# Kyubyong/dc_tts

Hardware: NVIDIA H100
Metric: mel_frames_per_sec (higher is better)
Workload: dtype f32 (decode: fp32 FMA; TextEnc/SSRN: fp16x2 split operands on wgmma, fp32 accumulate)

## Files before the change

### dc_tts_b200/csrc/api_synth.cu

```cuda
#include "api_internal.cuh"

namespace {

size_t decode_plane_halfs(H* h, int B, __half* base = nullptr, DecParams* set = nullptr) {
    const int T = h->hp.max_T;
    const std::vector<int> rows = audiodec_rows(h->audiodec, T);
    size_t off = 0;
    for (size_t i = 1; i < rows.size() && rows[i] > 1; ++i) {
        if (set) set->pl_hist[set->n_enc + i] = base + off;
        off += (size_t)B * h->audiodec[i].cin * 2 * (DEC_PL_PAD + T);
    }
    if (set) { set->pl_c1 = base + off; set->pl_rows = DEC_PL_PAD + T; }
    if (!h->audiodec.empty()) off += (size_t)(B + DEC_GMAX) * h->audiodec[0].cin * 2 * DEC_PL_PAD;
    return off;
}

}

void dctts::api::settle_decode_counts(H* h) {
    auto& D = h->dec;
    if (D.last_clusters > 0 && (D.last_moved_frames < 0 || D.frames_pending)) CUDA_CHECK(cudaDeviceSynchronize());
    if (D.last_clusters > 0 && D.last_moved_frames < 0) {
        std::vector<int> st(2 * (size_t)D.last_clusters);
        CUDA_CHECK(cudaMemcpy(st.data(), D.stats.p, st.size() * sizeof(int), cudaMemcpyDeviceToHost));
// ... 219 lines not shown
    }
    a.stages = std::min((occ2 || win.jptr) ? 2 : tc_stages_for(p.bn, bk, a.resid_tma, a.half), std::max(1, a.ntaps * a.kb_per_tap));
    if (debug)
        fprintf(stderr, "[tc] %s mode=%d ncta=%d bn=%d half=%d stages=%d nkb=%d tiles=%d TT=%d TB=%d L=%d B=%d\n", l.scope.c_str(),
                a.mode, p.ncta, a.bn, a.half, a.stages, a.ntaps * a.kb_per_tap, tiles, TT, TB, win.L, win.B);
    launch_conv_ln_tc(mAh, mAl, mWh, mWl, a.resid_tma ? io : nullptr, a, p.ncta, tiles, bk, lc.s); lc.count();
    if (debug) {
        cudaError_t e = cudaStreamSynchronize(lc.s);
        for (int c = 0; c < std::min(16, p.ncta * tiles); ++c)
            fprintf(stderr, "[tc]  cta %2d: start=%d tmem=0x%x nkb=%d tma=%d mma=%d acc_ready=%d published=%d combined=%d\n", c,
                    dbg_host[64 * c], dbg_host[64 * c + 1], dbg_host[64 * c + 2], dbg_host[64 * c + 3], dbg_host[64 * c + 4],
                    dbg_host[64 * c + 5], dbg_host[64 * c + 6], dbg_host[64 * c + 7]);
        {
            const int* d0 = dbg_host;
            auto dt = [&](int a_, int b_) { return (d0[b_] - d0[a_]) & 0x7fffffff; };
            fprintf(stderr, "[tc]  cta 0 cycles: setup %d | main loop %d | sweeps1+2 %d | cluster barrier %d | sweep3+stores %d | teardown %d | total %d\n",
                    dt(8, 9), dt(9, 10), dt(10, 11), dt(11, 12), dt(12, 13), dt(13, 14), dt(8, 14));
        }
        if (e != cudaSuccess) throw std::runtime_error(std::string("conv_ln_tc failed: ") + cudaGetErrorString(e));
    }
}

bool chain_tc_ok(H* h, const std::vector<LayerDev>& net) {
    if (h->tensor_path != 1) return false;
    for (auto& l : net) if (!l.tc.ok) return false;
    return true;
}

void run_chain_tc_planes(Launch& lc, const std::vector<LayerDev>& net, Planes cur, int which, int B, int L,
                         float* out, float* out_sig, int first_extra_shift, const float* in_inv, const int* lengths) {
    H* h = lc.h;
// ... 624 lines not shown
```

### dc_tts_b200/csrc/kernels_tc.cu

```cuda
#include "kernels_tc.cuh"
#include "numerics.cuh"
#include "tc_ptx.cuh"

#include <cstdlib>
#include <stdexcept>
#include <string>

namespace dctts {

using namespace ptx;

constexpr int TC_BM = 128;
constexpr int TC_THREADS = 384;
constexpr int TC_MAX_STAGES = 8;
constexpr int TC_AUX_BYTES = 256  + 3 * 512 * 4  + 128 * 16 ;
constexpr int TC_MAX_SMEM = 227 * 1024;

__device__ __forceinline__ void dbg_mark(int* dbg, int slot, int v) {
    if (dbg) {
        const int cta = blockIdx.y * gridDim.x + blockIdx.x;
        if (cta < 16) { reinterpret_cast<volatile int*>(dbg)[64 * cta + slot] = v; __threadfence_system(); }
    }
}

__device__ __forceinline__ void dbg_time(int* dbg, int slot) {
    if (dbg) dbg_mark(dbg, slot, (int)(clock64() & 0x7fffffff));
}

__device__ __forceinline__ void store_planes(const Planes& p, size_t row, int col, int C, const float (&o)[16]) {
    __half* hi = p.hi + row * p.ld + col;
    __half* lo = p.lo + row * p.ld + col;
    if (col + 16 <= p.ld) {
        split_store_f16<16>(o, hi, lo);
    } else {
#pragma unroll
        for (int i = 0; i < 16; ++i)
            if (col + i < C) split_f16(o[i], hi[i], lo[i]);
    }
}

__host__ __device__ inline int tc_acc_ld(int bn) { return bn + 4; }
__host__ __device__ inline int tc_ring_bytes(int stages, int stage_bytes, int bn) {
    const int ring = stages * stage_bytes;
    const int acc = TC_BM * tc_acc_ld(bn) * 4;
    return ((ring > acc ? ring : acc) + 1023) & ~1023;
}
__host__ __device__ constexpr int tc_max_cluster(int bn) { return bn == 144 ? 16 : 8; }
__host__ __device__ inline int tc_resid_bytes(int resid_tma, int half) { return resid_tma ? 2 * (half / 64) * 16384 : 0; }

template <int TC_BK, int BN>
__global__ void __launch_bounds__(TC_THREADS, 1)
conv_ln_tc_kernel(const __grid_constant__ CUtensorMap mapA_hi, const __grid_constant__ CUtensorMap mapA_lo,
                  const __grid_constant__ CUtensorMap mapW_hi, const __grid_constant__ CUtensorMap mapW_lo,
                  const __grid_constant__ CUtensorMap mapX_hi, const __grid_constant__ CUtensorMap mapX_lo,
                  const __grid_constant__ CUtensorMap mapO_hi, const __grid_constant__ CUtensorMap mapO_lo,
                  const TcArgs a) {
    extern __shared__ uint8_t smem_raw[];
    uint8_t* smem = reinterpret_cast<uint8_t*>((reinterpret_cast<uintptr_t>(smem_raw) + 1023) & ~uintptr_t(1023));
    pdl_launch_dependents();

    const int warp = threadIdx.x >> 5, lane = threadIdx.x & 31;
    const int wg = threadIdx.x >> 7;
    const bool epi = wg == 1;
    if (threadIdx.x == 0) dbg_time(a.dbg, 8);
    const int rank = (int)cluster_ctarank();
    const int ncta = (int)cluster_nctarank();
    const int nslices = ncta;
    constexpr int MAXC = tc_max_cluster(BN);
    constexpr int bn = BN;
    const int half = a.half;
    constexpr int TC_A_PLANE = TC_BM * TC_BK * 2;
    constexpr int SW = TC_BK * 2;
    constexpr int b_plane = bn * SW;
    constexpr int A_BYTES = 2 * TC_A_PLANE;
    constexpr int stage_bytes = A_BYTES + 2 * b_plane;
    const int stages = a.stages;
    const int nkb = a.ntaps * a.kb_per_tap;
    const int acc_ld = tc_acc_ld(bn);

    float* s_acc = reinterpret_cast<float*>(smem);
    uint8_t* rs = smem + tc_ring_bytes(stages, stage_bytes, bn);
    uint8_t* aux = rs + tc_resid_bytes(a.resid_tma, half);
    uint64_t* full_bar = reinterpret_cast<uint64_t*>(aux);
    uint64_t* empty_bar = full_bar + TC_MAX_STAGES;
    uint64_t* resid_bar = empty_bar + TC_MAX_STAGES;
    float* s_bias = reinterpret_cast<float*>(aux + 256);
    float* s_gam = s_bias + 512;
    float* s_bet = s_gam + 512;
    float4* s_part = reinterpret_cast<float4*>(s_bet + 512);

    pdl_wait();
    const int L = a.win.L;
    int t_end, t_lo;
    if (a.win.jptr) { t_end = __ldg(a.win.jptr); t_lo = max(0, t_end - a.win.R + 1); }
    else { t_end = L - 1; t_lo = 0; }
    int b0s, t0s;
// ... 19 lines not shown
        } else {
            int second = c >= half;
            int col = rank * half + (second ? c - half : c);
            bi = (a.mode == 1 && second) ? a.bias[a.C + col] : a.bias[col];
            g = second ? a.g2[col] : a.g1[col];
            be = second ? a.b2[col] : a.b1[col];
        }
        s_bias[c] = bi; s_gam[c] = g; s_bet[c] = be;
    }
    __syncthreads();
    if (threadIdx.x == 0) { dbg_mark(a.dbg, 0, 1); dbg_mark(a.dbg, 2, nkb); dbg_time(a.dbg, 9); }
    if (ncta > 1) { cluster_arrive(); cluster_wait(); }
    const uint16_t cta_mask = (uint16_t)((1u << ncta) - 1u);
    const int slice_rows = TC_BM / ncta;

    if (warp == 0) {
        if (lane == 0) {
            for (int kb = 0; kb < nkb; ++kb) {
                const int s = kb % stages;
                const uint32_t ph = (uint32_t)(kb / stages) & 1u;
                mbar_wait(&empty_bar[s], ph ^ 1u);
                mbar_expect_tx(&full_bar[s], (uint32_t)stage_bytes);
                uint8_t* st = smem + (size_t)s * stage_bytes;
                const int tap = kb / a.kb_per_tap, kc = kb - tap * a.kb_per_tap;
                const int tcoord = t0s + a.shifts[tap];
                if (mcast) {
                    const int off = rank * slice_rows * SW;
                    tma_load_3d_mc(&mapA_hi, &full_bar[s], st + off, kc * TC_BK, tcoord + rank * slice_rows, b0s, cta_mask);
                    tma_load_3d_mc(&mapA_lo, &full_bar[s], st + TC_A_PLANE + off, kc * TC_BK, tcoord + rank * slice_rows, b0s, cta_mask);
                } else {
                    tma_load_3d(&mapA_hi, &full_bar[s], st, kc * TC_BK, tcoord, b0s);
                    tma_load_3d(&mapA_lo, &full_bar[s], st + TC_A_PLANE, kc * TC_BK, tcoord, b0s);
                }
                tma_load_2d(&mapW_hi, &full_bar[s], st + A_BYTES, kb * TC_BK, rank * bn);
                tma_load_2d(&mapW_lo, &full_bar[s], st + A_BYTES + b_plane, kb * TC_BK, rank * bn);
            }
            dbg_mark(a.dbg, 3, nkb);
            if (a.resid_tma) {
                const int nbox = half / 64;
                mbar_expect_tx(resid_bar, (uint32_t)(2 * nbox * 16384));
                for (int i = 0; i < nbox; ++i) {
                    tma_load_3d(&mapX_hi, resid_bar, rs + i * 16384, rank * half + i * 64, t0s, b0s);
                    tma_load_3d(&mapX_lo, resid_bar, rs + (nbox + i) * 16384, rank * half + i * 64, t0s, b0s);
                }
            }
        }
        __syncwarp();
    } else if (wg >= 1) {
        const int mh = wg - 1;
        float acc[BN / 2];
#pragma unroll
        for (int i = 0; i < BN / 2; ++i) acc[i] = 0.f;
        auto release = [&](int s) {
            const int t = threadIdx.x & 127;
            if (mcast) { if (t < ncta) mbar_arrive_cluster(&empty_bar[s], (uint32_t)t); }
            else if (t == 0) mbar_arrive(&empty_bar[s]);
        };
        for (int kb = 0; kb < nkb; ++kb) {
            const int s = kb % stages;
            mbar_wait(&full_bar[s], (uint32_t)(kb / stages) & 1u);
            const uint32_t st = smem_u32(smem + (size_t)s * stage_bytes);
            const uint64_t dA_hi = gmma_desc_kmajor<SW>(st + mh * 64 * SW), dA_lo = gmma_desc_kmajor<SW>(st + TC_A_PLANE + mh * 64 * SW);
            const uint64_t dB_hi = gmma_desc_kmajor<SW>(st + A_BYTES), dB_lo = gmma_desc_kmajor<SW>(st + A_BYTES + b_plane);
            wg_fence();
#pragma unroll
            for (int k = 0; k < TC_BK / 16; ++k) {
                const uint64_t adv = (uint64_t)(k * 32 >> 4);
                wgmma_full<BN>(acc, dA_hi + adv, dB_hi + adv, (kb | k) != 0);
                wgmma_full<BN>(acc, dA_hi + adv, dB_lo + adv, 1u);
                wgmma_full<BN>(acc, dA_lo + adv, dB_hi + adv, 1u);
            }
            wg_commit();
            wg_wait<1>();
            if (kb > 0) release((kb - 1) % stages);
        }
        wg_wait<0>();
        wg_fence_regs(acc);
        if (threadIdx.x == 128) dbg_mark(a.dbg, 4, nkb);
        named_sync(1, 256);
        {
            const int w4 = (threadIdx.x >> 5) & 3;
            const int r0 = mh * 64 + w4 * 16 + (lane >> 2);
#pragma unroll
            for (int q = 0; q < BN / 8; ++q) {
                const int col = q * 8 + 2 * (lane & 3);
                *reinterpret_cast<float2*>(s_acc + (size_t)r0 * acc_ld + col) = make_float2(acc[q * 4], acc[q * 4 + 1]);
                *reinterpret_cast<float2*>(s_acc + (size_t)(r0 + 8) * acc_ld + col) = make_float2(acc[q * 4 + 2], acc[q * 4 + 3]);
            }
        }
        named_sync(1, 256);
    }
    if (epi) {
        const int r = threadIdx.x - 128;
        const float* arow = s_acc + (size_t)r * acc_ld;
        auto ld16 = [&](int c, float (&v)[16]) {
#pragma unroll
            for (int i = 0; i < 16; i += 4) {
                const float4 x = *reinterpret_cast<const float4*>(arow + c + i);
                v[i] = x.x; v[i + 1] = x.y; v[i + 2] = x.z; v[i + 3] = x.w;
            }
        };
        const int bi = r / a.TT, ti = r - bi * a.TT;
        const int n1 = (a.mode == 0) ? min(max(a.C - rank * bn, 0), bn) : half;
        if (r == 0) { dbg_mark(a.dbg, 5, 1); dbg_time(a.dbg, 10); }

        const int b = b0s + bi, t = t0s + ti;
        const bool row_ok = (b < a.win.B) && (t >= t_lo) && (t <= t_end) && (t < L);
        const bool live = !(a.lengths && b < a.win.B) ||
                          t < (min(max(__ldg(a.lengths + b), 0), L >> a.len_shift) << a.len_shift);
        const float in_s = (a.in_inv && b < a.win.B) ? __ldg(a.in_inv + b) : 1.f;
        const float inv_s = a.inv_scale * in_s;

        float s1, s2 = 0.f, q1, q2 = 0.f, m1, m2 = 0.f;
        {
            float piv = 0.f, S = 0.f, Q = 0.f;
            for (int c = 0; c < n1; c += 16) {
                float v[16];
                ld16(c, v);
                if (c == 0) piv = fmaf(v[0], inv_s, s_bias[0]);
#pragma unroll
                for (int i = 0; i < 16; ++i) {
                    const int cc = c + i;
                    if (cc < n1) { const float d = fmaf(v[i], inv_s, s_bias[cc]) - piv; S += d; Q = fmaf(d, d, Q); }
                }
            }
            const float n = (float)max(n1, 1);
            s1 = piv * (float)n1 + S; m1 = n1 > 0 ? s1 / n : 0.f; q1 = fmaxf(Q - S * S / n, 0.f);
        }
        if (a.mode != 0) {
            float piv = 0.f, S = 0.f, Q = 0.f;
            for (int c = 0; c < half; c += 16) {
                float v[16];
                ld16(half + c, v);
                if (c == 0) piv = fmaf(v[0], inv_s, s_bias[half]);
#pragma unroll
                for (int i = 0; i < 16; ++i) {
                    const int cc = c + i;
                    if (cc < half) { const float d = fmaf(v[i], inv_s, s_bias[half + cc]) - piv; S += d; Q = fmaf(d, d, Q); }
                }
            }
            s2 = piv * (float)half + S; m2 = s2 / (float)half; q2 = fmaxf(Q - S * S / (float)half, 0.f);
        }
        float mean1, rstd1, mean2 = 0.f, rstd2 = 0.f;
        if (ncta > 1) {
            s_part[r] = make_float4(s1, q1, s2, q2);
            if (r == 0) { dbg_mark(a.dbg, 6, 1); dbg_time(a.dbg, 11); }
            cluster_arrive();
            cluster_wait();
            if (r == 0) { dbg_mark(a.dbg, 7, 1); dbg_time(a.dbg, 12); }
            const uint32_t my_slot = smem_u32(&s_part[r]);
            float4 pv[MAXC];
#pragma unroll
            for (int p = 0; p < MAXC; ++p) pv[p] = (p < nslices) ? ld_cluster_f4(mapa(my_slot, (uint32_t)p)) : make_float4(0.f, 0.f, 0.f, 0.f);
            float S1 = 0.f, S2 = 0.f;
#pragma unroll
            for (int p = 0; p < MAXC; ++p) if (p < nslices) { S1 += pv[p].x; S2 += pv[p].z; }
            mean1 = S1 / (float)a.C; mean2 = S2 / (float)a.C;
            float M1 = 0.f, M2 = 0.f;
#pragma unroll
            for (int p = 0; p < MAXC; ++p) {
                if (p >= nslices) continue;
                const float4 v = pv[p];
                const int np = (a.mode == 0) ? min(max(a.C - p * bn, 0), bn) : half;
                if (np > 0) { float d = v.x / (float)np - mean1; M1 += v.y + (float)np * d * d; }
                if (a.mode != 0) { float d = v.z / (float)half - mean2; M2 += v.w + (float)half * d * d; }
            }
            rstd1 = 1.0f / sqrtf(M1 / (float)a.C + 1e-12f);
            rstd2 = 1.0f / sqrtf(M2 / (float)a.C + 1e-12f);
        } else {
            mean1 = m1; rstd1 = 1.0f / sqrtf(q1 / (float)a.C + 1e-12f);
            mean2 = m2; rstd2 = 1.0f / sqrtf(q2 / (float)a.C + 1e-12f);
        }

        {
            if (a.mode == 0) {
                const size_t row = (size_t)b * L + t;
                for (int c = 0; c < n1; c += 16) {
                    float v[16], o[16];
                    ld16(c, v);
                    const int col = rank * bn + c;
#pragma unroll
                    for (int i = 0; i < 16; ++i) {
                        float z = (fmaf(v[i], inv_s, s_bias[c + i]) - mean1) * rstd1 * s_gam[c + i] + s_bet[c + i];
                        if (a.act == 1) z = fmaxf(z, 0.f);
                        o[i] = (c + i < n1 && live) ? z : 0.f;
                    }
                    if (row_ok && a.out.hi) store_planes(a.out, row, col, a.C, o);
                    if (row_ok && a.out_f32) {
                        float* p = a.out_f32 + row * a.ld_f32 + col;
#pragma unroll
                        for (int i = 0; i < 16; ++i) if (c + i < n1) p[i] = o[i];
                    }
                    if (a.sig_f32 || a.sig.hi) {
#pragma unroll
                        for (int i = 0; i < 16; ++i) o[i] = (c + i < n1 && live) ? sigmoid_acc(o[i]) : 0.f;
                        if (row_ok && a.sig.hi) store_planes(a.sig, row, col, a.C, o);
                        if (row_ok && a.sig_f32) {
                            float* p = a.sig_f32 + row * a.ld_sig + col;
#pragma unroll
                            for (int i = 0; i < 16; ++i) if (c + i < n1) p[i] = o[i];
                        }
                    }
                }
            } else if (a.mode == 1) {
                const size_t row = (size_t)b * L + t;
                const int nbox = half / 64;
                if (a.resid_tma) mbar_wait(resid_bar, 0);
                for (int c = 0; c < half; c += 16) {
                    float v1[16], v2[16], o[16];
                    const int col = rank * half + c;
                    __align__(16) __half xh[16] = {};
                    __align__(16) __half xl[16] = {};
                    uint8_t* sh = rs + (c >> 6) * 16384 + r * 128;
                    uint8_t* sl = sh + nbox * 16384;
                    const int k0 = (((c & 63) >> 3) ^ (r & 7)) << 4, k1 = ((((c & 63) >> 3) + 1) ^ (r & 7)) << 4;
                    if (a.resid_tma) {
                        reinterpret_cast<uint4*>(xh)[0] = *reinterpret_cast<const uint4*>(sh + k0);
                        reinterpret_cast<uint4*>(xh)[1] = *reinterpret_cast<const uint4*>(sh + k1);
                        reinterpret_cast<uint4*>(xl)[0] = *reinterpret_cast<const uint4*>(sl + k0);
                        reinterpret_cast<uint4*>(xl)[1] = *reinterpret_cast<const uint4*>(sl + k1);
                    } else if (row_ok) {
                        const uint4* ph = reinterpret_cast<const uint4*>(a.X.hi + row * a.X.ld + col);
                        const uint4* pl = reinterpret_cast<const uint4*>(a.X.lo + row * a.X.ld + col);
                        reinterpret_cast<uint4*>(xh)[0] = __ldg(ph); reinterpret_cast<uint4*>(xh)[1] = __ldg(ph + 1);
                        reinterpret_cast<uint4*>(xl)[0] = __ldg(pl); reinterpret_cast<uint4*>(xl)[1] = __ldg(pl + 1);
                    }
                    ld16(c, v1);
                    ld16(half + c, v2);
#pragma unroll
                    for (int i = 0; i < 16; ++i) {
                        float z1 = (fmaf(v1[i], inv_s, s_bias[c + i]) - mean1) * rstd1 * s_gam[c + i] + s_bet[c + i];
                        float z2 = (fmaf(v2[i], inv_s, s_bias[half + c + i]) - mean2) * rstd2 * s_gam[half + c + i] + s_bet[half + c + i];
                        float h1 = sigmoid_acc(z1);
                        float x = join_f16(xh[i], xl[i]);
                        o[i] = live ? h1 * z2 + (1.0f - h1) * x : 0.f;
                    }
                    if (a.out_tma) {
                        __align__(16) __half oh[16];
                        __align__(16) __half ol[16];
#pragma unroll
                        for (int i = 0; i < 16; ++i) split_f16(o[i], oh[i], ol[i]);
                        *reinterpret_cast<uint4*>(sh + k0) = reinterpret_cast<const uint4*>(oh)[0];
                        *reinterpret_cast<uint4*>(sh + k1) = reinterpret_cast<const uint4*>(oh)[1];
                        *reinterpret_cast<uint4*>(sl + k0) = reinterpret_cast<const uint4*>(ol)[0];
                        *reinterpret_cast<uint4*>(sl + k1) = reinterpret_cast<const uint4*>(ol)[1];
                    } else if (row_ok && a.out.hi) {
                        store_planes(a.out, row, col, a.C, o);
                    }
                    if (row_ok && a.out_f32) {
                        float* p = a.out_f32 + row * a.ld_f32 + col;
#pragma unroll
                        for (int i = 0; i < 16; ++i) p[i] = o[i];
                    }
                }
                if (a.out_tma) {
                    fence_proxy_async_smem();
                    named_sync(2, 128);
                    if (r == 0) {
                        for (int i = 0; i < nbox; ++i) {
                            tma_store_3d(&mapO_hi, rs + i * 16384, rank * half + i * 64, t0s, b0s);
                            tma_store_3d(&mapO_lo, rs + (nbox + i) * 16384, rank * half + i * 64, t0s, b0s);
                        }
                        tma_store_commit_and_wait();
                    }
                }
            } else {
                const size_t row_e = (size_t)b * (2 * L) + 2 * (size_t)t;
                for (int hsel = 0; hsel < 2; ++hsel) {
                    const float mean = hsel ? mean2 : mean1, rstd = hsel ? rstd2 : rstd1;
                    for (int c = 0; c < half; c += 16) {
                        float v[16], o[16];
                        ld16(hsel * half + c, v);
                        const int col = rank * half + c;
#pragma unroll
                        for (int i = 0; i < 16; ++i) {
                            const int ac = hsel * half + c + i;
                            o[i] = live ? (fmaf(v[i], inv_s, s_bias[ac]) - mean) * rstd * s_gam[ac] + s_bet[ac] : 0.f;
                        }
                        if (row_ok && a.out.hi) store_planes(a.out, row_e + hsel, col, a.C, o);
                        if (row_ok && a.out_f32) {
                            float* p = a.out_f32 + (row_e + hsel) * a.ld_f32 + col;
#pragma unroll
                            for (int i = 0; i < 16; ++i) p[i] = o[i];
                        }
                    }
                }
            }
        }
        if (r == 0) dbg_time(a.dbg, 13);
    }

    if (ncta > 1) {
        if (!epi) { cluster_arrive(); cluster_wait(); }
        cluster_arrive();
        cluster_wait();
    }
    if (threadIdx.x == 0) dbg_time(a.dbg, 14);
}

__global__ void f32_to_planes_kernel(const float* __restrict__ x, int ldx, Planes p, long long rows, int C) {
    long long i = (long long)blockIdx.x * blockDim.x + threadIdx.x;
    long long total = rows * C;
    if (i >= total) return;
    long long r = i / C; int c = (int)(i - r * C);
    split_f16(x[r * ldx + c], p.hi[r * p.ld + c], p.lo[r * p.ld + c]);
}
__global__ void planes_to_f32_kernel(Planes p, float* __restrict__ y, int ldy, long long rows, int C) {
    long long i = (long long)blockIdx.x * blockDim.x + threadIdx.x;
// ... 94 lines not shown
    cuuint64_t strides[1] = {(cuuint64_t)Ktot * 2};
    cuuint32_t box[2] = {(cuuint32_t)bk, (cuuint32_t)bn};
    cuuint32_t estr[2] = {1, 1};
    CUresult r = encode_fn()(m, CU_TENSOR_MAP_DATA_TYPE_FLOAT16, 2, const_cast<__half*>(base), dims, strides, box, estr,
                             CU_TENSOR_MAP_INTERLEAVE_NONE, bk == 64 ? CU_TENSOR_MAP_SWIZZLE_128B : CU_TENSOR_MAP_SWIZZLE_64B, CU_TENSOR_MAP_L2_PROMOTION_L2_256B,
                             CU_TENSOR_MAP_FLOAT_OOB_FILL_NONE);
    if (r != CUDA_SUCCESS) throw std::runtime_error("cuTensorMapEncodeTiled(weights) failed: " + std::to_string((int)r));
}

int tc_bk() {
    return 32;
}

static size_t conv_ln_smem(int stages, int bn, int half, int resid_tma, int bk) {
    const int stage = 2 * TC_BM * bk * 2 + 2 * bn * bk * 2;
    return (size_t)tc_ring_bytes(stages, stage, bn) + tc_resid_bytes(resid_tma, half) + TC_AUX_BYTES + 1024;
}

int tc_stages_for(int bn, int bk, int resid_tma, int half) {
    int s = TC_MAX_STAGES;
    while (s > 2 && conv_ln_smem(s, bn, half, resid_tma, bk) > (size_t)TC_MAX_SMEM) --s;
    return s;
}

typedef void (*ConvLnKernel)(const CUtensorMap, const CUtensorMap, const CUtensorMap, const CUtensorMap, const CUtensorMap,
                             const CUtensorMap, const CUtensorMap, const CUtensorMap, const TcArgs);
template <int BK>
static ConvLnKernel conv_ln_kernel_bn(int bn) {
    switch (bn) {
        case 64: return conv_ln_tc_kernel<BK, 64>;
        case 80: return conv_ln_tc_kernel<BK, 80>;
// ... 29 lines not shown
    cudaLaunchAttribute at[1];
    at[0].id = cudaLaunchAttributeClusterDimension;
    at[0].val.clusterDim.x = (unsigned)ncta; at[0].val.clusterDim.y = 1; at[0].val.clusterDim.z = 1;
    cfg.attrs = at; cfg.numAttrs = 1;
    int n = 0;
    if (cudaOccupancyMaxActiveClusters(&n, kern, &cfg) != cudaSuccess) { cudaGetLastError(); return 0; }
    return n;
}

void launch_conv_ln_tc(const CUtensorMap& a_hi, const CUtensorMap& a_lo, const CUtensorMap& w_hi,
                       const CUtensorMap& w_lo, const CUtensorMap* io, const TcArgs& a, int ncta, int ctas_y, int bk,
                       cudaStream_t s) {
    if (ncta > tc_max_cluster(a.bn))
        throw std::runtime_error("conv_ln_tc: a cluster of " + std::to_string(ncta) + " CTAs at " + std::to_string(a.bn) +
                                 " columns (16 at 144 columns, else 8 at most)");
    const ConvLnKernel kern = conv_ln_kernel_ready(bk, a.bn);
    const size_t smem = conv_ln_smem(a.stages, a.bn, a.half, a.resid_tma, bk);
    if (smem > (size_t)TC_MAX_SMEM) throw std::runtime_error("conv_ln_tc: shared memory budget exceeded");
    cudaLaunchConfig_t cfg{};
    cfg.gridDim = dim3((unsigned)ncta, (unsigned)ctas_y, 1);
    cfg.blockDim = dim3(TC_THREADS, 1, 1);
    cfg.dynamicSmemBytes = smem;
    cfg.stream = s;
    cudaLaunchAttribute at[2];
    at[0].id = cudaLaunchAttributeClusterDimension;
    at[0].val.clusterDim.x = (unsigned)ncta; at[0].val.clusterDim.y = 1; at[0].val.clusterDim.z = 1;
    at[1].id = cudaLaunchAttributeProgrammaticStreamSerialization;
    at[1].val.programmaticStreamSerializationAllowed = 1;
    cfg.attrs = at; cfg.numAttrs = pdl_enabled() ? 2 : 1;
    if (a.resid_tma && !io) throw std::runtime_error("conv_ln_tc: residual TMA needs the X / out tensor maps");
// ... 10 lines not shown
```

### dc_tts_b200/csrc/tc_ptx.cuh

```cuda
#pragma once
#include <cuda_runtime.h>
#include <stdint.h>

namespace dctts { namespace ptx {

__device__ __forceinline__ uint32_t smem_u32(const void* p) {
    return static_cast<uint32_t>(__cvta_generic_to_shared(p));
}
__device__ __forceinline__ bool elect_one() {
    uint32_t pred = 0;
    asm volatile("{\n\t.reg .pred P;\n\telect.sync _|P, 0xffffffff;\n\tselp.u32 %0, 1, 0, P;\n\t}" : "=r"(pred));
    return pred != 0;
}

__device__ __forceinline__ void mbar_init(uint64_t* bar, uint32_t count) {
    asm volatile("mbarrier.init.shared::cta.b64 [%0], %1;" :: "r"(smem_u32(bar)), "r"(count));
}
__device__ __forceinline__ void fence_mbar_init() { asm volatile("fence.mbarrier_init.release.cluster;" ::: "memory"); }
__device__ __forceinline__ void mbar_expect_tx(uint64_t* bar, uint32_t bytes) {
    asm volatile("mbarrier.arrive.expect_tx.shared::cta.b64 _, [%0], %1;" :: "r"(smem_u32(bar)), "r"(bytes) : "memory");
}
__device__ __forceinline__ bool mbar_try_wait(uint64_t* bar, uint32_t parity) {
    uint32_t ok;
    asm volatile(
// ... 130 lines not shown
    return d;
}

__device__ __forceinline__ void mbar_arrive(uint64_t* bar) {
    asm volatile("mbarrier.arrive.shared::cta.b64 _, [%0];" :: "r"(smem_u32(bar)) : "memory");
}
__device__ __forceinline__ uint32_t mapa(uint32_t smem_addr, uint32_t rank);
__device__ __forceinline__ void mbar_arrive_cluster(uint64_t* bar, uint32_t rank) {
    asm volatile("mbarrier.arrive.release.cluster.shared::cluster.b64 _, [%0];" :: "r"(mapa(smem_u32(bar), rank)) : "memory");
}
__device__ __forceinline__ void mbar_arrive_remote(uint64_t* bar, uint32_t rank) {
    asm volatile("mbarrier.arrive.shared::cluster.b64 _, [%0];" :: "r"(mapa(smem_u32(bar), rank)) : "memory");
}
__device__ __forceinline__ void named_sync(int id, int n) { asm volatile("bar.sync %0, %1;" :: "r"(id), "r"(n) : "memory"); }

__device__ __forceinline__ uint32_t cluster_ctarank() { uint32_t r; asm volatile("mov.u32 %0, %%cluster_ctarank;" : "=r"(r)); return r; }
__device__ __forceinline__ uint32_t cluster_nctarank() { uint32_t r; asm volatile("mov.u32 %0, %%cluster_nctarank;" : "=r"(r)); return r; }
__device__ __forceinline__ void cluster_arrive() { asm volatile("barrier.cluster.arrive.release.aligned;" ::: "memory"); }
__device__ __forceinline__ void cluster_wait() { asm volatile("barrier.cluster.wait.acquire.aligned;" ::: "memory"); }
__device__ __forceinline__ uint32_t mapa(uint32_t smem_addr, uint32_t rank) {
    uint32_t r;
    asm volatile("mapa.shared::cluster.u32 %0, %1, %2;" : "=r"(r) : "r"(smem_addr), "r"(rank));
    return r;
}
__device__ __forceinline__ float4 ld_cluster_f4(uint32_t addr) {
    float4 v;
    asm volatile("ld.shared::cluster.v4.f32 {%0, %1, %2, %3}, [%4];" : "=f"(v.x), "=f"(v.y), "=f"(v.z), "=f"(v.w) : "r"(addr) : "memory");
    return v;
}
__device__ __forceinline__ void st_cluster_f4(uint32_t addr, float a, float b, float c, float d) {
// ... 5 lines not shown
```

Measured before the change: 136,800.

## Compute LayerNorm epilogue directly from wgmma register fragments instead of smem staging

The conv+LayerNorm tensor-core kernel used to dump its accumulators to a shared-memory tile and have one warpgroup redo row statistics and normalisation per row. Now both MMA warpgroups apply bias, compute row statistics with quad shuffles, normalise and store directly from their register fragments. Stores use quad transposes to form 16-byte writes. This removes the smem round trip and the accumulator tile from the smem budget, which may allow more pipeline stages. Register reallocation via setmaxnreg gives the consumer warpgroups more registers; it adds shuffle work and a new constraint that hc/transposed modes need half == bn/2.

```diff
diff --git a/dc_tts_b200/csrc/api_synth.cu b/dc_tts_b200/csrc/api_synth.cu
--- a/dc_tts_b200/csrc/api_synth.cu
+++ b/dc_tts_b200/csrc/api_synth.cu
@@ -257,7 +257,7 @@
         {
             const int* d0 = dbg_host;
             auto dt = [&](int a_, int b_) { return (d0[b_] - d0[a_]) & 0x7fffffff; };
-            fprintf(stderr, "[tc]  cta 0 cycles: setup %d | main loop %d | sweeps1+2 %d | cluster barrier %d | sweep3+stores %d | teardown %d | total %d\n",
+            fprintf(stderr, "[tc]  cta 0 cycles: setup %d | main loop %d | statistics %d | cluster barrier %d | normalise+stores %d | teardown %d | total %d\n",
                     dt(8, 9), dt(9, 10), dt(10, 11), dt(11, 12), dt(12, 13), dt(13, 14), dt(8, 14));
         }
         if (e != cudaSuccess) throw std::runtime_error(std::string("conv_ln_tc failed: ") + cudaGetErrorString(e));
diff --git a/dc_tts_b200/csrc/kernels_tc.cu b/dc_tts_b200/csrc/kernels_tc.cu
--- a/dc_tts_b200/csrc/kernels_tc.cu
+++ b/dc_tts_b200/csrc/kernels_tc.cu
@@ -27,24 +27,82 @@
     if (dbg) dbg_mark(dbg, slot, (int)(clock64() & 0x7fffffff));
 }
 
-__device__ __forceinline__ void store_planes(const Planes& p, size_t row, int col, int C, const float (&o)[16]) {
-    __half* hi = p.hi + row * p.ld + col;
-    __half* lo = p.lo + row * p.ld + col;
-    if (col + 16 <= p.ld) {
-        split_store_f16<16>(o, hi, lo);
-    } else {
-#pragma unroll
-        for (int i = 0; i < 16; ++i)
-            if (col + i < C) split_f16(o[i], hi[i], lo[i]);
-    }
-}
-
-__host__ __device__ inline int tc_acc_ld(int bn) { return bn + 4; }
-__host__ __device__ inline int tc_ring_bytes(int stages, int stage_bytes, int bn) {
-    const int ring = stages * stage_bytes;
-    const int acc = TC_BM * tc_acc_ld(bn) * 4;
-    return ((ring > acc ? ring : acc) + 1023) & ~1023;
-}
+
+template <int G0, int NG, int R>
+__device__ __forceinline__ void row_stats(const float (&v)[R], int h, int j, int n, float& s, float& m2) {
+    const float piv = __shfl_sync(0xffffffffu, v[4 * G0 + 2 * h], (threadIdx.x & 31) & ~3);
+    float S = 0.f, Q = 0.f;
+#pragma unroll
+    for (int k = 0; k < NG; ++k)
+#pragma unroll
+        for (int e = 0; e < 2; ++e)
+            if (8 * k + 2 * j + e < n) { const float d = v[4 * (G0 + k) + 2 * h + e] - piv; S += d; Q = fmaf(d, d, Q); }
+#pragma unroll
+    for (int m = 1; m < 4; m <<= 1) { S += __shfl_xor_sync(0xffffffffu, S, m); Q += __shfl_xor_sync(0xffffffffu, Q, m); }
+    s = piv * (float)n + S;
+    m2 = fmaxf(Q - S * S / (float)max(n, 1), 0.f);
+}
+
+__device__ __forceinline__ void quad_transpose(uint32_t (&x)[4], int j) {
+#pragma unroll
+    for (int m = 2; m > 0; m >>= 1) {
+        const bool up = (j & m) != 0;
+#pragma unroll
+        for (int k = 0; k < 4; ++k) {
+            if (k & m) continue;
+            const uint32_t r = __shfl_xor_sync(0xffffffffu, up ? x[k] : x[k ^ m], m);
+            if (up) x[k] = r; else x[k ^ m] = r;
+        }
+    }
+}
+
+__device__ __forceinline__ uint32_t h2_bits(__half2 v) { return *reinterpret_cast<uint32_t*>(&v); }
+
+template <int G0, int NG, int R>
+__device__ __forceinline__ void store_planes_frag(const Planes& p, size_t row, int col0, const float (&v)[R], int h, int j,
+                                                  bool ok) {
+    __half* hi = p.hi + row * p.ld;
+    __half* lo = p.lo + row * p.ld;
+#pragma unroll
+    for (int k = 0; k + 4 <= NG; k += 4) {
+        uint32_t xh[4], xl[4];
+#pragma unroll
+        for (int i = 0; i < 4; ++i) {
+            const int q = G0 + k + i;
+            __half2 a, b;
+            split_f16x2(make_float2(v[4 * q + 2 * h], v[4 * q + 2 * h + 1]), a, b);
+            xh[i] = h2_bits(a); xl[i] = h2_bits(b);
+        }
+        quad_transpose(xh, j);
+        quad_transpose(xl, j);
+        const int col = col0 + 8 * (k + j);
+        if (ok && col + 8 <= p.ld) {
+            *reinterpret_cast<uint4*>(hi + col) = make_uint4(xh[0], xh[1], xh[2], xh[3]);
+            *reinterpret_cast<uint4*>(lo + col) = make_uint4(xl[0], xl[1], xl[2], xl[3]);
+        }
+    }
+#pragma unroll
+    for (int k = NG & ~3; k < NG; ++k) {
+        const int q = G0 + k, col = col0 + 8 * k + 2 * j;
+        __half2 a, b;
+        split_f16x2(make_float2(v[4 * q + 2 * h], v[4 * q + 2 * h + 1]), a, b);
+        if (ok && col + 2 <= p.ld) { *reinterpret_cast<__half2*>(hi + col) = a; *reinterpret_cast<__half2*>(lo + col) = b; }
+    }
+}
+
+template <int G0, int NG, int R>
+__device__ __forceinline__ void store_f32_frag(float* dst, int col0, int n, const float (&v)[R], int h, int j) {
+#pragma unroll
+    for (int k = 0; k < NG; ++k) {
+        const int c = 8 * k + 2 * j;
+        const float x0 = v[4 * (G0 + k) + 2 * h], x1 = v[4 * (G0 + k) + 2 * h + 1];
+        float* d = dst + col0 + c;
+        if (c + 1 < n && (reinterpret_cast<uintptr_t>(d) & 7) == 0) *reinterpret_cast<float2*>(d) = make_float2(x0, x1);
+        else { if (c < n) d[0] = x0; if (c + 1 < n) d[1] = x1; }
+    }
+}
+
+__host__ __device__ inline int tc_ring_bytes(int stages, int stage_bytes) { return (stages * stage_bytes + 1023) & ~1023; }
 __host__ __device__ constexpr int tc_max_cluster(int bn) { return bn == 144 ? 16 : 8; }
 __host__ __device__ inline int tc_resid_bytes(int resid_tma, int half) { return resid_tma ? 2 * (half / 64) * 16384 : 0; }
 
@@ -56,12 +114,11 @@
                   const __grid_constant__ CUtensorMap mapO_hi, const __grid_constant__ CUtensorMap mapO_lo,
                   const TcArgs a) {
     extern __shared__ uint8_t smem_raw[];
-    uint8_t* smem = reinterpret_cast<uint8_t*>((reinterpret_cast<uintptr_t>(smem_raw) + 1023) & ~uintptr_t(1023));
+    uint8_t* smem = smem_raw + ((1024u - (smem_u32(smem_raw) & 1023u)) & 1023u);
     pdl_launch_dependents();
 
     const int warp = threadIdx.x >> 5, lane = threadIdx.x & 31;
     const int wg = threadIdx.x >> 7;
-    const bool epi = wg == 1;
     if (threadIdx.x == 0) dbg_time(a.dbg, 8);
     const int rank = (int)cluster_ctarank();
     const int ncta = (int)cluster_nctarank();
@@ -69,6 +126,7 @@
     constexpr int MAXC = tc_max_cluster(BN);
     constexpr int bn = BN;
     const int half = a.half;
+    constexpr int HALF = BN / 2, NG = BN / 8, HG = BN / 16;
     constexpr int TC_A_PLANE = TC_BM * TC_BK * 2;
     constexpr int SW = TC_BK * 2;
     constexpr int b_plane = bn * SW;
@@ -76,10 +134,8 @@
     constexpr int stage_bytes = A_BYTES + 2 * b_plane;
     const int stages = a.stages;
     const int nkb = a.ntaps * a.kb_per_tap;
-    const int acc_ld = tc_acc_ld(bn);
-
-    float* s_acc = reinterpret_cast<float*>(smem);
-    uint8_t* rs = smem + tc_ring_bytes(stages, stage_bytes, bn);
+
+    uint8_t* rs = smem + tc_ring_bytes(stages, stage_bytes);
     uint8_t* aux = rs + tc_resid_bytes(a.resid_tma, half);
     uint64_t* full_bar = reinterpret_cast<uint64_t*>(aux);
     uint64_t* empty_bar = full_bar + TC_MAX_STAGES;
@@ -129,8 +185,9 @@
     const uint16_t cta_mask = (uint16_t)((1u << ncta) - 1u);
     const int slice_rows = TC_BM / ncta;
 
-    if (warp == 0) {
-        if (lane == 0) {
+    if (wg == 0) {
+        setmaxnreg_dec<40>();
+        if (warp == 0 && lane == 0) {
             for (int kb = 0; kb < nkb; ++kb) {
                 const int s = kb % stages;
                 const uint32_t ph = (uint32_t)(kb / stages) & 1u;
@@ -161,7 +218,8 @@
             }
         }
         __syncwarp();
-    } else if (wg >= 1) {
+    } else {
+        setmaxnreg_inc<232>();
         const int mh = wg - 1;
         float acc[BN / 2];
 #pragma unroll
@@ -191,222 +249,197 @@
         }
         wg_wait<0>();
         wg_fence_regs(acc);
-        if (threadIdx.x == 128) dbg_mark(a.dbg, 4, nkb);
-        named_sync(1, 256);
-        {
-            const int w4 = (threadIdx.x >> 5) & 3;
-            const int r0 = mh * 64 + w4 * 16 + (lane >> 2);
-#pragma unroll
-            for (int q = 0; q < BN / 8; ++q) {
-                const int col = q * 8 + 2 * (lane & 3);
-                *reinterpret_cast<float2*>(s_acc + (size_t)r0 * acc_ld + col) = make_float2(acc[q * 4], acc[q * 4 + 1]);
-                *reinterpret_cast<float2*>(s_acc + (size_t)(r0 + 8) * acc_ld + col) = make_float2(acc[q * 4 + 2], acc[q * 4 + 3]);
-            }
-        }
-        named_sync(1, 256);
-    }
-    if (epi) {
-        const int r = threadIdx.x - 128;
-        const float* arow = s_acc + (size_t)r * acc_ld;
-        auto ld16 = [&](int c, float (&v)[16]) {
-#pragma unroll
-            for (int i = 0; i < 16; i += 4) {
-                const float4 x = *reinterpret_cast<const float4*>(arow + c + i);
-                v[i] = x.x; v[i + 1] = x.y; v[i + 2] = x.z; v[i + 3] = x.w;
-            }
-        };
-        const int bi = r / a.TT, ti = r - bi * a.TT;
-        const int n1 = (a.mode == 0) ? min(max(a.C - rank * bn, 0), bn) : half;
-        if (r == 0) { dbg_mark(a.dbg, 5, 1); dbg_time(a.dbg, 10); }
-
-        const int b = b0s + bi, t = t0s + ti;
-        const bool row_ok = (b < a.win.B) && (t >= t_lo) && (t <= t_end) && (t < L);
-        const bool live = !(a.lengths && b < a.win.B) ||
-                          t < (min(max(__ldg(a.lengths + b), 0), L >> a.len_shift) << a.len_shift);
-        const float in_s = (a.in_inv && b < a.win.B) ? __ldg(a.in_inv + b) : 1.f;
-        const float inv_s = a.inv_scale * in_s;
-
-        float s1, s2 = 0.f, q1, q2 = 0.f, m1, m2 = 0.f;
-        {
-            float piv = 0.f, S = 0.f, Q = 0.f;
-            for (int c = 0; c < n1; c += 16) {
-                float v[16];
-                ld16(c, v);
-                if (c == 0) piv = fmaf(v[0], inv_s, s_bias[0]);
-#pragma unroll
-                for (int i = 0; i < 16; ++i) {
-                    const int cc = c + i;
-                    if (cc < n1) { const float d = fmaf(v[i], inv_s, s_bias[cc]) - piv; S += d; Q = fmaf(d, d, Q); }
-                }
-            }
-            const float n = (float)max(n1, 1);
-            s1 = piv * (float)n1 + S; m1 = n1 > 0 ? s1 / n : 0.f; q1 = fmaxf(Q - S * S / n, 0.f);
-        }
-        if (a.mode != 0) {
-            float piv = 0.f, S = 0.f, Q = 0.f;
-            for (int c = 0; c < half; c += 16) {
-                float v[16];
-                ld16(half + c, v);
-                if (c == 0) piv = fmaf(v[0], inv_s, s_bias[half]);
-#pragma unroll
-                for (int i = 0; i < 16; ++i) {
-                    const int cc = c + i;
-                    if (cc < half) { const float d = fmaf(v[i], inv_s, s_bias[half + cc]) - piv; S += d; Q = fmaf(d, d, Q); }
-                }
-            }
-            s2 = piv * (float)half + S; m2 = s2 / (float)half; q2 = fmaxf(Q - S * S / (float)half, 0.f);
-        }
-        float mean1, rstd1, mean2 = 0.f, rstd2 = 0.f;
+        if (threadIdx.x == 128) { dbg_mark(a.dbg, 4, nkb); dbg_mark(a.dbg, 5, 1); dbg_time(a.dbg, 10); }
+
+        const int j = lane & 3;
+        const int rt = mh * 64 + (warp & 3) * 16 + (lane >> 2);
+        int bb[2], tt[2];
+        bool ok[2], live[2];
+        float inv_s[2];
+#pragma unroll
+        for (int h = 0; h < 2; ++h) {
+            const int r = rt + 8 * h, bi = r / a.TT;
+            const int b = b0s + bi, t = t0s + r - bi * a.TT;
+            bb[h] = b; tt[h] = t;
+            ok[h] = (b < a.win.B) && (t >= t_lo) && (t <= t_end) && (t < L);
+            live[h] = !(a.lengths && b < a.win.B) || t < (min(max(__ldg(a.lengths + b), 0), L >> a.len_shift) << a.len_shift);
+            inv_s[h] = a.inv_scale * ((a.in_inv && b < a.win.B) ? __ldg(a.in_inv + b) : 1.f);
+        }
+#pragma unroll
+        for (int q = 0; q < NG; ++q) {
+            const float2 bi2 = *reinterpret_cast<const float2*>(s_bias + 8 * q + 2 * j);
+#pragma unroll
+            for (int h = 0; h < 2; ++h) {
+                acc[4 * q + 2 * h] = fmaf(acc[4 * q + 2 * h], inv_s[h], bi2.x);
+                acc[4 * q + 2 * h + 1] = fmaf(acc[4 * q + 2 * h + 1], inv_s[h], bi2.y);
+            }
+        }
+        const int n1 = (a.mode == 0) ? min(max(a.C - rank * bn, 0), bn) : HALF;
+
+        float s1[2], q1[2], s2[2] = {0.f, 0.f}, q2[2] = {0.f, 0.f};
+#pragma unroll
+        for (int h = 0; h < 2; ++h) {
+            if (a.mode == 0) row_stats<0, NG>(acc, h, j, n1, s1[h], q1[h]);
+            else { row_stats<0, HG>(acc, h, j, HALF, s1[h], q1[h]); row_stats<HG, HG>(acc, h, j, HALF, s2[h], q2[h]); }
+        }
+        float mean1[2], rstd1[2], mean2[2] = {0.f, 0.f}, rstd2[2] = {0.f, 0.f};
         if (ncta > 1) {
-            s_part[r] = make_float4(s1, q1, s2, q2);
-            if (r == 0) { dbg_mark(a.dbg, 6, 1); dbg_time(a.dbg, 11); }
+            if (j == 0) {
+                s_part[rt] = make_float4(s1[0], q1[0], s2[0], q2[0]);
+                s_part[rt + 8] = make_float4(s1[1], q1[1], s2[1], q2[1]);
+            }
+            if (threadIdx.x == 128) { dbg_mark(a.dbg, 6, 1); dbg_time(a.dbg, 11); }
             cluster_arrive();
             cluster_wait();
-            if (r == 0) { dbg_mark(a.dbg, 7, 1); dbg_time(a.dbg, 12); }
-            const uint32_t my_slot = smem_u32(&s_part[r]);
-            float4 pv[MAXC];
-#pragma unroll
-            for (int p = 0; p < MAXC; ++p) pv[p] = (p < nslices) ? ld_cluster_f4(mapa(my_slot, (uint32_t)p)) : make_float4(0.f, 0.f, 0.f, 0.f);
-            float S1 = 0.f, S2 = 0.f;
-#pragma unroll
-            for (int p = 0; p < MAXC; ++p) if (p < nslices) { S1 += pv[p].x; S2 += pv[p].z; }
-            mean1 = S1 / (float)a.C; mean2 = S2 / (float)a.C;
-            float M1 = 0.f, M2 = 0.f;
-#pragma unroll
-            for (int p = 0; p < MAXC; ++p) {
-                if (p >= nslices) continue;
-                const float4 v = pv[p];
-                const int np = (a.mode == 0) ? min(max(a.C - p * bn, 0), bn) : half;
-                if (np > 0) { float d = v.x / (float)np - mean1; M1 += v.y + (float)np * d * d; }
-                if (a.mode != 0) { float d = v.z / (float)half - mean2; M2 += v.w + (float)half * d * d; }
-            }
-            rstd1 = 1.0f / sqrtf(M1 / (float)a.C + 1e-12f);
-            rstd2 = 1.0f / sqrtf(M2 / (float)a.C + 1e-12f);
+            if (threadIdx.x == 128) { dbg_mark(a.dbg, 7, 1); dbg_time(a.dbg, 12); }
+#pragma unroll
+            for (int h = 0; h < 2; ++h) {
+                const uint32_t my_slot = smem_u32(&s_part[rt + 8 * h]);
+                float4 pv[MAXC];
+#pragma unroll
+                for (int p = 0; p < MAXC; ++p) pv[p] = (p < nslices) ? ld_cluster_f4(mapa(my_slot, (uint32_t)p)) : make_float4(0.f, 0.f, 0.f, 0.f);
+                float S1 = 0.f, S2 = 0.f;
+#pragma unroll
+                for (int p = 0; p < MAXC; ++p) if (p < nslices) { S1 += pv[p].x; S2 += pv[p].z; }
+                mean1[h] = S1 / (float)a.C; mean2[h] = S2 / (float)a.C;
+                float M1 = 0.f, M2 = 0.f;
+#pragma unroll
+                for (int p = 0; p < MAXC; ++p) {
+                    if (p >= nslices) continue;
+                    const float4 v = pv[p];
+                    const int np = (a.mode == 0) ? min(max(a.C - p * bn, 0), bn) : HALF;
+                    if (np > 0) { float d = v.x / (float)np - mean1[h]; M1 += v.y + (float)np * d * d; }
+                    if (a.mode != 0) { float d = v.z / (float)HALF - mean2[h]; M2 += v.w + (float)HALF * d * d; }
+                }
+                rstd1[h] = 1.0f / sqrtf(M1 / (float)a.C + 1e-12f);
+                rstd2[h] = 1.0f / sqrtf(M2 / (float)a.C + 1e-12f);
+            }
         } else {
-            mean1 = m1; rstd1 = 1.0f / sqrtf(q1 / (float)a.C + 1e-12f);
-            mean2 = m2; rstd2 = 1.0f / sqrtf(q2 / (float)a.C + 1e-12f);
-        }
-
-        {
-            if (a.mode == 0) {
-                const size_t row = (size_t)b * L + t;
-                for (int c = 0; c < n1; c += 16) {
-                    float v[16], o[16];
-                    ld16(c, v);
-                    const int col = rank * bn + c;
-#pragma unroll
-                    for (int i = 0; i < 16; ++i) {
-                        float z = (fmaf(v[i], inv_s, s_bias[c + i]) - mean1) * rstd1 * s_gam[c + i] + s_bet[c + i];
+#pragma unroll
+            for (int h = 0; h < 2; ++h) {
+                mean1[h] = n1 > 0 ? s1[h] / (float)max(n1, 1) : 0.f; rstd1[h] = 1.0f / sqrtf(q1[h] / (float)a.C + 1e-12f);
+                mean2[h] = s2[h] / (float)HALF; rstd2[h] = 1.0f / sqrtf(q2[h] / (float)a.C + 1e-12f);
+            }
+        }
+
+        if (a.mode == 0) {
+#pragma unroll
+            for (int q = 0; q < NG; ++q)
+#pragma unroll
+                for (int h = 0; h < 2; ++h)
+#pragma unroll
+                    for (int e = 0; e < 2; ++e) {
+                        const int c = 8 * q + 2 * j + e;
+                        float z = (acc[4 * q + 2 * h + e] - mean1[h]) * rstd1[h] * s_gam[c] + s_bet[c];
                         if (a.act == 1) z = fmaxf(z, 0.f);
-                        o[i] = (c + i < n1 && live) ? z : 0.f;
+                        acc[4 * q + 2 * h + e] = (c < n1 && live[h]) ? z : 0.f;
                     }
-                    if (row_ok && a.out.hi) store_planes(a.out, row, col, a.C, o);
-                    if (row_ok && a.out_f32) {
-                        float* p = a.out_f32 + row * a.ld_f32 + col;
-#pragma unroll
-                        for (int i = 0; i < 16; ++i) if (c + i < n1) p[i] = o[i];
+            const int col0 = rank * bn;
+#pragma unroll
+            for (int h = 0; h < 2; ++h) {
+                const size_t row = (size_t)bb[h] * L + tt[h];
+                if (a.out.hi) store_planes_frag<0, NG>(a.out, row, col0, acc, h, j, ok[h]);
+                if (ok[h] && a.out_f32) store_f32_frag<0, NG>(a.out_f32 + row * a.ld_f32, col0, n1, acc, h, j);
+            }
+            if (a.sig_f32 || a.sig.hi) {
+#pragma unroll
+                for (int h = 0; h < 2; ++h)
+#pragma unroll
+                    for (int q = 0; q < NG; ++q)
+#pragma unroll
+                        for (int e = 0; e < 2; ++e) {
+                            const int c = 8 * q + 2 * j + e;
+                            acc[4 * q + 2 * h + e] = (c < n1 && live[h]) ? sigmoid_acc(acc[4 * q + 2 * h + e]) : 0.f;
+                        }
+#pragma unroll
+                for (int h = 0; h < 2; ++h) {
+                    const size_t row = (size_t)bb[h] * L + tt[h];
+                    if (a.sig.hi) store_planes_frag<0, NG>(a.sig, row, col0, acc, h, j, ok[h]);
+                    if (ok[h] && a.sig_f32) store_f32_frag<0, NG>(a.sig_f32 + row * a.ld_sig, col0, n1, acc, h, j);
+                }
+            }
+        } else if (a.mode == 1) {
+            const int nbox = HALF / 64;
+            if (a.resid_tma) mbar_wait(resid_bar, 0);
+#pragma unroll
+            for (int q = 0; q < HG; ++q) {
+#pragma unroll
+                for (int h = 0; h < 2; ++h) {
+                    const int r = rt + 8 * h;
+                    const size_t row = (size_t)bb[h] * L + tt[h];
+                    const int c = 8 * q + 2 * j;
+                    uint8_t* sh = rs + (q >> 3) * 16384 + r * 128 + ((((q & 7) ^ (r & 7)) << 4) | (4 * j));
+                    uint8_t* sl = sh + nbox * 16384;
+                    __half2 xh = __float2half2_rn(0.f), xl = xh;
+                    if (a.resid_tma) {
+                        xh = *reinterpret_cast<const __half2*>(sh);
+                        xl = *reinterpret_cast<const __half2*>(sl);
+                    } else if (ok[h]) {
+                        xh = __ldg(reinterpret_cast<const __half2*>(a.X.hi + row * a.X.ld + rank * HALF + c));
+                        xl = __ldg(reinterpret_cast<const __half2*>(a.X.lo + row * a.X.ld + rank * HALF + c));
                     }
-                    if (a.sig_f32 || a.sig.hi) {
-#pragma unroll
-                        for (int i = 0; i < 16; ++i) o[i] = (c + i < n1 && live) ? sigmoid_acc(o[i]) : 0.f;
-                        if (row_ok && a.sig.hi) store_planes(a.sig, row, col, a.C, o);
-                        if (row_ok && a.sig_f32) {
-                            float* p = a.sig_f32 + row * a.ld_sig + col;
-#pragma unroll
-                            for (int i = 0; i < 16; ++i) if (c + i < n1) p[i] = o[i];
-                        }
-                    }
-                }
-            } else if (a.mode == 1) {
-                const size_t row = (size_t)b * L + t;
-                const int nbox = half / 64;
-                if (a.resid_tma) mbar_wait(resid_bar, 0);
-                for (int c = 0; c < half; c += 16) {
-                    float v1[16], v2[16], o[16];
-                    const int col = rank * half + c;
-                    __align__(16) __half xh[16] = {};
-                    __align__(16) __half xl[16] = {};
-                    uint8_t* sh = rs + (c >> 6) * 16384 + r * 128;
-                    uint8_t* sl = sh + nbox * 16384;
-                    const int k0 = (((c & 63) >> 3) ^ (r & 7)) << 4, k1 = ((((c & 63) >> 3) + 1) ^ (r & 7)) << 4;
-                    if (a.resid_tma) {
-                        reinterpret_cast<uint4*>(xh)[0] = *reinterpret_cast<const uint4*>(sh + k0);
-                        reinterpret_cast<uint4*>(xh)[1] = *reinterpret_cast<const uint4*>(sh + k1);
-                        reinterpret_cast<uint4*>(xl)[0] = *reinterpret_cast<const uint4*>(sl + k0);
-                        reinterpret_cast<uint4*>(xl)[1] = *reinterpret_cast<const uint4*>(sl + k1);
-                    } else if (row_ok) {
-                        const uint4* ph = reinterpret_cast<const uint4*>(a.X.hi + row * a.X.ld + col);
-                        const uint4* pl = reinterpret_cast<const uint4*>(a.X.lo + row * a.X.ld + col);
-                        reinterpret_cast<uint4*>(xh)[0] = __ldg(ph); reinterpret_cast<uint4*>(xh)[1] = __ldg(ph + 1);
-                        reinterpret_cast<uint4*>(xl)[0] = __ldg(pl); reinterpret_cast<uint4*>(xl)[1] = __ldg(pl + 1);
-                    }
-                    ld16(c, v1);
-                    ld16(half + c, v2);
-#pragma unroll
-                    for (int i = 0; i < 16; ++i) {
-                        float z1 = (fmaf(v1[i], inv_s, s_bias[c + i]) - mean1) * rstd1 * s_gam[c + i] + s_bet[c + i];
-                        float z2 = (fmaf(v2[i], inv_s, s_bias[half + c + i]) - mean2) * rstd2 * s_gam[half + c + i] + s_bet[half + c + i];
-                        float h1 = sigmoid_acc(z1);
-                        float x = join_f16(xh[i], xl[i]);
-                        o[i] = live ? h1 * z2 + (1.0f - h1) * x : 0.f;
+#pragma unroll
+                    for (int e = 0; e < 2; ++e) {
+                        const float z1 = (acc[4 * q + 2 * h + e] - mean1[h]) * rstd1[h] * s_gam[c + e] + s_bet[c + e];
+                        const float z2 = (acc[4 * (q + HG) + 2 * h + e] - mean2[h]) * rstd2[h] * s_gam[HALF + c + e] + s_bet[HALF + c + e];
+                        const float h1 = sigmoid_acc(z1);
+                        const float x = e ? join_f16(__high2half(xh), __high2half(xl)) : join_f16(__low2half(xh), __low2half(xl));
+                        acc[4 * q + 2 * h + e] = live[h] ? h1 * z2 + (1.0f - h1) * x : 0.f;
                     }
                     if (a.out_tma) {
-                        __align__(16) __half oh[16];
-                        __align__(16) __half ol[16];
-#pragma unroll
-                        for (int i = 0; i < 16; ++i) split_f16(o[i], oh[i], ol[i]);
-                        *reinterpret_cast<uint4*>(sh + k0) = reinterpret_cast<const uint4*>(oh)[0];
-                        *reinterpret_cast<uint4*>(sh + k1) = reinterpret_cast<const uint4*>(oh)[1];
-                        *reinterpret_cast<uint4*>(sl + k0) = reinterpret_cast<const uint4*>(ol)[0];
-                        *reinterpret_cast<uint4*>(sl + k1) = reinterpret_cast<const uint4*>(ol)[1];
-                    } else if (row_ok && a.out.hi) {
-                        store_planes(a.out, row, col, a.C, o);
+                        __half2 oh, ol;
+                        split_f16x2(make_float2(acc[4 * q + 2 * h], acc[4 * q + 2 * h + 1]), oh, ol);
+                        *reinterpret_cast<__half2*>(sh) = oh;
+                        *reinterpret_cast<__half2*>(sl) = ol;
                     }
-                    if (row_ok && a.out_f32) {
-                        float* p = a.out_f32 + row * a.ld_f32 + col;
-#pragma unroll
-                        for (int i = 0; i < 16; ++i) p[i] = o[i];
+                }
+            }
+#pragma unroll
+            for (int h = 0; h < 2; ++h) {
+                const size_t row = (size_t)bb[h] * L + tt[h];
+                if (!a.out_tma && a.out.hi) store_planes_frag<0, HG>(a.out, row, rank * HALF, acc, h, j, ok[h]);
+                if (ok[h] && a.out_f32) store_f32_frag<0, HG>(a.out_f32 + row * a.ld_f32, rank * HALF, HALF, acc, h, j);
+            }
+            if (a.out_tma) {
+                fence_proxy_async_smem();
+                named_sync(1, 256);
+                if (threadIdx.x == 128) {
+                    for (int i = 0; i < nbox; ++i) {
+                        tma_store_3d(&mapO_hi, rs + i * 16384, rank * HALF + i * 64, t0s, b0s);
+                        tma_store_3d(&mapO_lo, rs + (nbox + i) * 16384, rank * HALF + i * 64, t0s, b0s);
                     }
-                }
-                if (a.out_tma) {
-                    fence_proxy_async_smem();
-                    named_sync(2, 128);
-                    if (r == 0) {
-                        for (int i = 0; i < nbox; ++i) {
-                            tma_store_3d(&mapO_hi, rs + i * 16384, rank * half + i * 64, t0s, b0s);
-                            tma_store_3d(&mapO_lo, rs + (nbox + i) * 16384, rank * half + i * 64, t0s, b0s);
-                        }
-                        tma_store_commit_and_wait();
+                    tma_store_commit_and_wait();
+                }
+            }
+        } else {
+#pragma unroll
+            for (int q = 0; q < NG; ++q)
+#pragma unroll
+                for (int h = 0; h < 2; ++h)
+#pragma unroll
+                    for (int e = 0; e < 2; ++e) {
+                        const int c = 8 * q + 2 * j + e;
+                        const float mean = q < HG ? mean1[h] : mean2[h], rstd = q < HG ? rstd1[h] : rstd2[h];
+                        acc[4 * q + 2 * h + e] = live[h] ? (acc[4 * q + 2 * h + e] - mean) * rstd * s_gam[c] + s_bet[c] : 0.f;
                     }
-                }
-            } else {
-                const size_t row_e = (size_t)b * (2 * L) + 2 * (size_t)t;
-                for (int hsel = 0; hsel < 2; ++hsel) {
-                    const float mean = hsel ? mean2 : mean1, rstd = hsel ? rstd2 : rstd1;
-                    for (int c = 0; c < half; c += 16) {
-                        float v[16], o[16];
-                        ld16(hsel * half + c, v);
-                        const int col = rank * half + c;
-#pragma unroll
-                        for (int i = 0; i < 16; ++i) {
-                            const int ac = hsel * half + c + i;
-                            o[i] = live ? (fmaf(v[i], inv_s, s_bias[ac]) - mean) * rstd * s_gam[ac] + s_bet[ac] : 0.f;
-                        }
-                        if (row_ok && a.out.hi) store_planes(a.out, row_e + hsel, col, a.C, o);
-                        if (row_ok && a.out_f32) {
-                            float* p = a.out_f32 + (row_e + hsel) * a.ld_f32 + col;
-#pragma unroll
-                            for (int i = 0; i < 16; ++i) p[i] = o[i];
-                        }
-                    }
-                }
-            }
-        }
-        if (r == 0) dbg_time(a.dbg, 13);
+#pragma unroll
+            for (int h = 0; h < 2; ++h) {
+                const size_t row_e = (size_t)bb[h] * (2 * L) + 2 * (size_t)tt[h];
+                if (a.out.hi) {
+                    store_planes_frag<0, HG>(a.out, row_e, rank * HALF, acc, h, j, ok[h]);
+                    store_planes_frag<HG, HG>(a.out, row_e + 1, rank * HALF, acc, h, j, ok[h]);
+                }
+                if (ok[h] && a.out_f32) {
+                    store_f32_frag<0, HG>(a.out_f32 + row_e * a.ld_f32, rank * HALF, HALF, acc, h, j);
+                    store_f32_frag<HG, HG>(a.out_f32 + (row_e + 1) * a.ld_f32, rank * HALF, HALF, acc, h, j);
+                }
+            }
+        }
+        if (threadIdx.x == 128) dbg_time(a.dbg, 13);
     }
 
     if (ncta > 1) {
-        if (!epi) { cluster_arrive(); cluster_wait(); }
+        if (wg == 0) { cluster_arrive(); cluster_wait(); }
         cluster_arrive();
         cluster_wait();
     }
@@ -531,7 +564,7 @@
 
 static size_t conv_ln_smem(int stages, int bn, int half, int resid_tma, int bk) {
     const int stage = 2 * TC_BM * bk * 2 + 2 * bn * bk * 2;
-    return (size_t)tc_ring_bytes(stages, stage, bn) + tc_resid_bytes(resid_tma, half) + TC_AUX_BYTES + 1024;
+    return (size_t)tc_ring_bytes(stages, stage) + tc_resid_bytes(resid_tma, half) + TC_AUX_BYTES + 1024;
 }
 
 int tc_stages_for(int bn, int bk, int resid_tma, int half) {
@@ -591,6 +624,7 @@
     if (ncta > tc_max_cluster(a.bn))
         throw std::runtime_error("conv_ln_tc: a cluster of " + std::to_string(ncta) + " CTAs at " + std::to_string(a.bn) +
                                  " columns (16 at 144 columns, else 8 at most)");
+    if (a.mode != 0 && 2 * a.half != a.bn) throw std::runtime_error("conv_ln_tc: hc and transposed blocks hold two halves of bn / 2 columns");
     const ConvLnKernel kern = conv_ln_kernel_ready(bk, a.bn);
     const size_t smem = conv_ln_smem(a.stages, a.bn, a.half, a.resid_tma, bk);
     if (smem > (size_t)TC_MAX_SMEM) throw std::runtime_error("conv_ln_tc: shared memory budget exceeded");
diff --git a/dc_tts_b200/csrc/tc_ptx.cuh b/dc_tts_b200/csrc/tc_ptx.cuh
--- a/dc_tts_b200/csrc/tc_ptx.cuh
+++ b/dc_tts_b200/csrc/tc_ptx.cuh
@@ -168,6 +168,11 @@
 }
 __device__ __forceinline__ void named_sync(int id, int n) { asm volatile("bar.sync %0, %1;" :: "r"(id), "r"(n) : "memory"); }
 
+template <int N>
+__device__ __forceinline__ void setmaxnreg_dec() { asm volatile("setmaxnreg.dec.sync.aligned.u32 %0;" :: "n"(N)); }
+template <int N>
+__device__ __forceinline__ void setmaxnreg_inc() { asm volatile("setmaxnreg.inc.sync.aligned.u32 %0;" :: "n"(N)); }
+
 __device__ __forceinline__ uint32_t cluster_ctarank() { uint32_t r; asm volatile("mov.u32 %0, %%cluster_ctarank;" : "=r"(r)); return r; }
 __device__ __forceinline__ uint32_t cluster_nctarank() { uint32_t r; asm volatile("mov.u32 %0, %%cluster_nctarank;" : "=r"(r)); return r; }
 __device__ __forceinline__ void cluster_arrive() { asm volatile("barrier.cluster.arrive.release.aligned;" ::: "memory"); }
```

New measurement: 141,100, median of 6. +3.2%, better.
